# fwilliams/point-cloud-utils

Hardware: AMD Instinct MI355X
Metric: query-points/s, Chamfer 1M-vs-1M fp32 (higher is better)
Workload: dtype f32

## Files before the change

### point_cloud_utils_amd/csrc/grid.h

```cpp
#pragma once
#include "pcu_types.h"

#ifndef PCU_SORT_THREADS
#define PCU_SORT_THREADS 1024
#endif

namespace pcu {

constexpr int kBlock = 256;

template <typename T>
__device__ __forceinline__ T wave_min(T v) {
#pragma unroll
    for (int o = 32; o > 0; o >>= 1) { T w = __shfl_xor(v, o, 64); v = w < v ? w : v; }
    return v;
}
template <typename T>
__device__ __forceinline__ T wave_max(T v) {
#pragma unroll
    for (int o = 32; o > 0; o >>= 1) { T w = __shfl_xor(v, o, 64); v = w > v ? w : v; }
    return v;
}

template <int CTRL, int ROW_MASK, int BANK_MASK, bool BOUND>
// ... 389 lines not shown
template <typename T>
__global__ __launch_bounds__(kBlock) void k_scatter(const T* __restrict__ pts, int n, const unsigned* __restrict__ cell_of,
                                                    const unsigned* rank, const unsigned* __restrict__ cell_start,
                                                    Pt4<T>* __restrict__ sorted) {
    const int i = blockIdx.x * kBlock + threadIdx.x;
    if (i >= n) return;
    if (cell_of[i] == 0xffffffffu) return;
    Pt4<T> p;
    p.x = pts[3 * (size_t)i]; p.y = pts[3 * (size_t)i + 1]; p.z = pts[3 * (size_t)i + 2]; p.idx = i;
    const unsigned pos = cell_start[cell_of[i]] + rank[i];
    sorted[pos] = p;
    put_xyz(sorted, n, pos, p);
}

constexpr int kBkThreads = 1024;
#ifndef PCU_BK_PTS
#define PCU_BK_PTS 8
#endif
constexpr int kBkPts = PCU_BK_PTS;
constexpr int kBkBlockPts = kBkThreads * kBkPts;
constexpr int kBkMaxBuckets = 8192;
constexpr int kBkMaxCellsPerBucket = 4096;
constexpr int kSortThreads = PCU_SORT_THREADS;
constexpr int kSortIters = 8;
constexpr unsigned kLargeBucket = kSortThreads * kSortIters;
#ifndef PCU_BUCKET_PTS
#define PCU_BUCKET_PTS 4096
#endif
#ifndef PCU_STAGE_RECS
#define PCU_STAGE_RECS 4352
#endif
constexpr int kBucketPts = PCU_BUCKET_PTS;
constexpr int kStageRecs = PCU_STAGE_RECS;

template <typename T> struct RawRec;
template <> struct RawRec<float>  { typedef unsigned __attribute__((ext_vector_type(4))) type; };
template <> struct RawRec<double> { typedef unsigned long long __attribute__((ext_vector_type(4))) type; };

template <typename T>
__device__ __forceinline__ unsigned cell_linear(const GridParams<T>& g, T x, T y, T z) {
    const int cx = grid_cell(g, 0, x), cy = grid_cell(g, 1, y), cz = grid_cell(g, 2, z);
    return (unsigned)row_run_lo(g.G[0], grid_row(g.G[1], cy, cz), cx, cx);
}

__device__ __forceinline__ unsigned count_rank(unsigned* counter, unsigned key, bool valid) {
    const unsigned long long act = __ballot(valid);
    if (act == 0) return 0;
// ... 571 lines not shown
```

### point_cloud_utils_amd/csrc/grid2.h

```cpp
#pragma once
#include "grid.h"

namespace pcu {

constexpr int kPrepSamples = 1024;
constexpr int kXPartStride = 8;
constexpr int kStagedMaxBuckets = 2048;
constexpr int kFillWords = 2 * kStagedMaxBuckets + 8;

template <typename T>
struct CellMap {
    T org[3], inv_h; int G[3];
    __device__ __forceinline__ explicit CellMap(const GridParams<T>& g) {
#pragma unroll
        for (int j = 0; j < 3; ++j) { org[j] = uniform(g.org[j]); G[j] = uniform(g.G[j]); }
        inv_h = uniform(g.inv_h);
    }
    __device__ __forceinline__ unsigned cell(T x, T y, T z) const {
        const int cx = cell_coord(x, org[0], inv_h, G[0]), cy = cell_coord(y, org[1], inv_h, G[1]), cz = cell_coord(z, org[2], inv_h, G[2]);
        return (unsigned)row_run_lo(G[0], grid_row(G[1], cy, cz), cx, cx);
    }
};

__device__ __forceinline__ unsigned hash32(unsigned x) { x ^= x >> 16; x *= 0x7feb352du; x ^= x >> 15; x *= 0x846ca68bu; x ^= x >> 16; return x; }
// ... 189 lines not shown
            const bool valid = base + j * kBkThreads + tid < n;
            bk[j] = cm.cell(px[j], py[j], pz[j]) >> shift;
            rk[j] = count_rank(s_cnt, bk[j], valid);
            const T v[3] = {px[j], py[j], pz[j]};
#pragma unroll
            for (int c = 0; c < 3; ++c) {
                const bool fin = (v[c] < (T)0 ? -v[c] : v[c]) <= Limits<T>::max_v;
                lo[c] = (valid && fin && v[c] < lo[c]) ? v[c] : lo[c];
                hi[c] = (valid && fin && v[c] > hi[c]) ? v[c] : hi[c];
                if (valid && !fin) nf |= v[c] != v[c] ? 1u : (v[c] > (T)0 ? (2u << c) : (16u << c));
            }
        }
#pragma unroll
        for (int c = 0; c < 3; ++c) { s_col[c * kBkThreads + tid] = lo[c]; s_col[(3 + c) * kBkThreads + tid] = hi[c]; }
        const unsigned wf = wave_or63(nf);
        if (wf && lane == 63) atomicOr(&s_nf, wf);
    }
    __syncthreads();
    P3_PROF(2);
    if (wave < 6) {
        const T r = fold_column<T, kBkThreads>(s_col + wave * kBkThreads, wave < 3 ? 0 : 1, lane);
        if (lane == 63) a.xpartial[(size_t)bid * kXPartStride + wave] = r;
    } else if (tid == 6 * 64) a.xpartial[(size_t)bid * kXPartStride + 6] = (T)s_nf;
    {
        static_assert(kStagedMaxBuckets == 2 * kBkThreads, "two buckets per thread");
        const int i0 = 2 * tid;
        const unsigned c0 = i0 < NB ? s_cnt[i0] : 0u, c1 = i0 + 1 < NB ? s_cnt[i0 + 1] : 0u;
        unsigned total;
        const unsigned ex = block_exclusive_scan_nt<kBkThreads>(c0 + c1, &total);
        if (i0 < NB) s_lbase[i0] = ex;
        if (i0 + 1 < NB) s_lbase[i0 + 1] = ex + c0;
#pragma unroll
        for (int q = 0; q < 2; ++q) {
            const int i = i0 + q; const unsigned c = q ? c1 : c0;
            if (i < NB && c) {
                const unsigned pad = (c + 7u) & ~7u;
                const unsigned at = (unsigned)atomicAdd(&a.fill[i], ((unsigned long long)c << 32) | (unsigned long long)pad);
                if (at + pad > cap) { *a.ovf = 1ull; s_gbase[i] = 0xffffffffu; }
                else s_gbase[i] = (unsigned)i * cap + at;
            }
        }
    }
    __syncthreads();
    P3_PROF(3);
    typedef typename RawRec<T>::type Raw;
#pragma unroll
    for (int j = 0; j < PTS; ++j) {
        const int i = base + j * kBkThreads + tid;
        if (i < n) { Pt4<T> p; p.x = px[j]; p.y = py[j]; p.z = pz[j]; p.idx = i; s_stage[s_lbase[bk[j]] + rk[j]] = p; }
    }
    __syncthreads();
    P3_PROF(4);
    Pt4<T> hole; hole.x = hole.y = hole.z = (T)0; hole.idx = -1;
    for (int r0 = 0; r0 * 1024 + wave < NB; ++r0) {
        const int mine = wave + 16 * (64 * r0 + lane);
        const unsigned mc = mine < NB ? s_cnt[mine] : 0u, ml = mine < NB ? s_lbase[mine] : 0u, mg = mine < NB ? s_gbase[mine] : 0u;
        const int nk = min(64, (NB - wave - 1024 * r0 + 15) / 16);
        for (int k = 0; k < nk; ++k) {
            const unsigned c = (unsigned)__shfl((int)mc, k, 64);
            if (c == 0) continue;
            const unsigned lb = (unsigned)__shfl((int)ml, k, 64), gb = (unsigned)__shfl((int)mg, k, 64);
            if (gb == 0xffffffffu) continue;
            const unsigned pad = (c + 7u) & ~7u;
            for (unsigned l = (unsigned)lane; l < pad; l += 64u) {
                Pt4<T> rec = hole;
                if (l < c) rec = s_stage[lb + l];
                a.tmp[gb + l] = rec;
            }
        }
    }
    P3_PROF(5);
    if (prof) { asm volatile("s_waitcnt vmcnt(0)" ::: "memory"); P3_PROF(6); if (tid == 0) atomicAdd((unsigned long long*)&prof[15], 1ull); }
#undef P3_PROF
}

template <typename T>
__device__ __forceinline__ void fold_xpartials(const Build2Side<T>& a) {
    __shared__ T s_lo[kSortThreads / 64][3], s_hi[kSortThreads / 64][3];
    __shared__ unsigned s_nf[kSortThreads / 64];
    const int tid = threadIdx.x, lane = tid & 63, wave = tid >> 6;
    __shared__ int s_stale;
    if (tid == 0) s_stale = 0;
    if (a.geo_out) {
        extern __shared__ __attribute__((aligned(32))) unsigned char s_dyn[];
        T* const s_col = reinterpret_cast<T*>(s_dyn);
        __shared__ T s_fin[13];
        __shared__ GridParams<T> s_fresh;
        T rng6[6];
        const SampleOf<T> smp = sample_request<T>(a, a.n, tid);
        layout_from_sample<T>(a, a.n, smp, s_col, s_fin, &s_fresh, rng6);
// ... 34 lines not shown
    for (int j = 0; j < 3; ++j) {
        const T p = wave_min63(lo[j]), q = wave_max63(hi[j]);
        if (lane == 63) { s_lo[wave][j] = p; s_hi[wave][j] = q; }
    }
    { const unsigned m = wave_or63(nf); if (lane == 63) s_nf[wave] = m; }
    __syncthreads();
    if (tid != 0) return;
    GridParams<T>* gp = a.gp;
    unsigned m = 0;
    for (int w = 0; w < kSortThreads / 64; ++w) m |= s_nf[w];
    const unsigned pinf = (m >> 1) & 7u, ninf = (m >> 4) & 7u;
    gp->nonfinite = ((m & 1u) ? kNfNaN : 0) | ((pinf & ninf) ? kNfBothInf : 0) | ((pinf | ninf) ? kNfAnyInf : 0) | (int)(m << 8);
    for (int j = 0; j < 3; ++j) {
        T p = s_lo[0][j], q = s_hi[0][j];
        for (int w = 1; w < kSortThreads / 64; ++w) { p = s_lo[w][j] < p ? s_lo[w][j] : p; q = s_hi[w][j] > q ? s_hi[w][j] : q; }
        if (!(p <= q)) { p = 0; q = 0; }
        gp->gmin[j] = p; gp->gmax[j] = q;
    }
    gp->has_large = (*a.ovf ? 2 : 0) | (s_stale ? kGeoStale : 0);
    if (a.n_large) *a.n_large = 0u;
    put_sentinels(a.sorted, a.n);
}

constexpr int kRegIters = (kStageRecs + kSortThreads - 1) / kSortThreads;
template <typename T, bool FAST>
__device__ __forceinline__ void sort2_body(const int b, const Build2Side<T>& a, const int cnt_cap, const unsigned s, const unsigned pf, const unsigned nvalid,
                                           unsigned* const s_cnt, Pt4<T>* const s_stage, unsigned* const s_w, unsigned long long* const s_q, long long t_prev) {
    GridParams<T>* const gp = a.gp;
    const CellMap<T> cm(*gp);
    const int ncells = uniform(gp->ncells);
    const int shift = a.shift, CB = 1 << shift;
    const int NB = (ncells + CB - 1) >> shift;
    const int tid = threadIdx.x, lane = tid & 63, wave = tid >> 6;
    long long* const prof = a.prof;
#define S2_PROF(slot) do { if (prof && tid == 0) { const long long t_now = wall_clock64(); atomicAdd((unsigned long long*)&prof[slot], (unsigned long long)(t_now - t_prev)); t_prev = t_now; } } while (0)
    const unsigned cap = a.cap;
    const unsigned c0 = (unsigned)b << shift;
    const int ncl = min(CB, ncells - (int)c0);
    const unsigned e = s + nvalid;
    const Pt4<T>* const slot = a.tmp + (size_t)b * cap;
    const unsigned lastp = pf ? pf - 1u : 0u;
    typedef typename RawRec<T>::type Raw;
    constexpr int kIters = FAST ? kRegIters : kSortIters;
    constexpr int kSortBatch = 4;
    Raw recs[FAST ? kRegIters : 1];
    unsigned rr[kIters];
    if (FAST) {
        const Raw* const rslot = reinterpret_cast<const Raw*>(slot);
#pragma unroll
        for (int u = 0; u < kRegIters; ++u) recs[u] = rslot[min((unsigned)(u * kSortThreads + tid), lastp)];
#pragma unroll
        for (int u = 0; u < kRegIters; ++u) {
            const unsigned p = (unsigned)(u * kSortThreads + tid);
            const Pt4<T>& rec = reinterpret_cast<const Pt4<T>&>(recs[u]);
            rr[u] = 0xffffffffu;
            if (p < pf && rec.idx >= 0) {
                const unsigned c = cm.cell(rec.x, rec.y, rec.z) - c0;
                rr[u] = (c << 16) | atomicAdd(&s_cnt[c], 1u);
            }
        }
    } else {
#pragma unroll
        for (int it0 = 0; it0 < kIters; it0 += kSortBatch) {
            Pt4<T> rec[kSortBatch];
            const bool batch_on = (unsigned)(it0 * kSortThreads) < pf;
            if (batch_on) {
#pragma unroll
                for (int u = 0; u < kSortBatch; ++u) rec[u] = slot[min((unsigned)((it0 + u) * kSortThreads + tid), lastp)];
            }
#pragma unroll
            for (int u = 0; u < kSortBatch; ++u) {
                const unsigned p = (unsigned)((it0 + u) * kSortThreads + tid);
                rr[it0 + u] = 0xffffffffu;
// ... 46 lines not shown
    T* const xyz = xyz_of(a.sorted, n_pts);
    int* const idx32 = idx32_of(a.sorted, n_pts);
    if (!FAST) {
#pragma unroll
        for (int it0 = 0; it0 < kIters; it0 += kSortBatch) {
            if (!((unsigned)(it0 * kSortThreads) < pf)) break;
            Pt4<T> rec[kSortBatch];
#pragma unroll
            for (int u = 0; u < kSortBatch; ++u) rec[u] = slot[min((unsigned)((it0 + u) * kSortThreads + tid), lastp)];
#pragma unroll
            for (int u = 0; u < kSortBatch; ++u) {
                const unsigned r = rr[it0 + u];
                if (r != 0xffffffffu) {
                    const unsigned pos = s + s_cnt[r >> 16] + (r & 0xffffu);
                    if (a.want_pt4) a.sorted[pos] = rec[u];
                    put_xyz(a.sorted, n_pts, pos, rec[u]);
                }
            }
        }
        return;
    }
    constexpr unsigned V = 16 / sizeof(T);
    T* const st = reinterpret_cast<T*>(s_stage);
    int* const sidx = reinterpret_cast<int*>(st + (V + 3 * kStageRecs + V - 1) / V * V);
    static_assert(((V + 3 * kStageRecs + V - 1) / V * V) * sizeof(T) + (size_t)kStageRecs * 4 <= (size_t)kStageRecs * sizeof(Pt4<T>) + 64, "both streams fit the stage (bucket_sort_lds_bytes)");
    const unsigned phase = (unsigned)((3ull * (unsigned long long)s) & (V - 1));
    {
#pragma unroll
        for (int u = 0; u < kRegIters; ++u) {
            const unsigned r = rr[u];
            if (r != 0xffffffffu) {
                const Pt4<T>& rec = reinterpret_cast<const Pt4<T>&>(recs[u]);
                const unsigned pos = s_cnt[r >> 16] + (r & 0xffffu);
                T* const o = st + phase + 3u * pos;
                o[0] = rec.x; o[1] = rec.y; o[2] = rec.z; sidx[pos] = (int)rec.idx;
            }
        }
    }
    __syncthreads();
    S2_PROF(3);
    for (unsigned i = tid; i < nvalid; i += kSortThreads) {
        const int id = sidx[i];
        idx32[s + i] = id;
        if (a.want_pt4) { Pt4<T> r; const T* const o = st + phase + 3u * i; r.x = o[0]; r.y = o[1]; r.z = o[2]; r.idx = id; a.sorted[s + i] = r; }
    }
    {
        const unsigned end = phase + 3u * nvalid;
        T* const out = xyz + (3 * (size_t)s - phase);
        typedef typename RawRec<float>::type Raw16;
        const unsigned v0 = (phase + V - 1) / V, v1 = end / V;
        for (unsigned c = v0 + tid; c < v1; c += kSortThreads)
            reinterpret_cast<Raw16*>(out)[c] = reinterpret_cast<const Raw16*>(st)[c];
        if (tid < V) {
            const unsigned La = phase + tid;
            if (La < min(v0 * V, end)) out[La] = st[La];
            const unsigned Lb = max(v1 * V, v0 * V) + tid;
            if (v1 >= v0 && Lb < end) out[Lb] = st[Lb];
        }
    }
    S2_PROF(4);
    if (prof) { asm volatile("s_waitcnt vmcnt(0)" ::: "memory"); S2_PROF(5); if (tid == 0) atomicAdd((unsigned long long*)&prof[7], 1ull); }
#undef S2_PROF
}

template <typename T>
__device__ __forceinline__ void sort2_bucket(const int b, const Build2Side<T>& a, const int cnt_cap) {
    extern __shared__ __attribute__((aligned(32))) unsigned char s_dyn[];
    unsigned* const s_cnt = reinterpret_cast<unsigned*>(s_dyn);
    Pt4<T>* const s_stage = reinterpret_cast<Pt4<T>*>(s_dyn + (size_t)cnt_cap * 4);
    __shared__ unsigned s_w[kSortThreads / 64 + 1];
    __shared__ unsigned long long s_q[kSortThreads / 64];
    if (*a.ovf) return;
    const int CB = 1 << a.shift;
    const int NB = (uniform(a.gp->ncells) + CB - 1) >> a.shift;
    if (b >= NB) return;
    const int tid = threadIdx.x, lane = tid & 63, wave = tid >> 6;
    long long t_prev = a.prof ? wall_clock64() : 0;
    unsigned s;
    {
        unsigned part = 0;
        for (int i = tid; i < b; i += kSortThreads) part += (unsigned)(a.fill[i] >> 32);
#pragma unroll
        for (int o = 32; o > 0; o >>= 1) part += __shfl_xor(part, o, 64);
        if (lane == 0) s_w[wave] = part;
        for (int i = tid; i < CB; i += kSortThreads) s_cnt[i] = 0u;
        __syncthreads();
        s = 0;
        for (int w = 0; w < kSortThreads / 64; ++w) s += s_w[w];
        __syncthreads();
    }
    if (a.prof && tid == 0) { const long long t_now = wall_clock64(); atomicAdd((unsigned long long*)&a.prof[0], (unsigned long long)(t_now - t_prev)); t_prev = t_now; }
    const unsigned long long fw = a.fill[b];
    const unsigned pf = min((unsigned)fw, a.cap), nvalid = (unsigned)(fw >> 32);
    static_assert(kSortThreads * kSortIters >= kLargeBucket, "one trip per record of a full slot");
    if (pf <= (unsigned)(kRegIters * kSortThreads) && nvalid <= (unsigned)kStageRecs) sort2_body<T, true>(b, a, cnt_cap, s, pf, nvalid, s_cnt, s_stage, s_w, s_q, t_prev);
    else sort2_body<T, false>(b, a, cnt_cap, s, pf, nvalid, s_cnt, s_stage, s_w, s_q, t_prev);
}

template <typename T>
__global__ __launch_bounds__(kSortThreads) void k_bucket_sort2(const Build2Args<T> p, int nb0, int nb1, int cnt_cap, int nfold) {
    const int bid = (int)blockIdx.x;
    if (bid < nfold) { fold_xpartials<T>(p.a[bid]); return; }
    const int b = bid - nfold;
    const int side = b >= nb0 ? 1 : 0;
    sort2_bucket<T>(side ? b - nb0 : b, p.a[side], cnt_cap);
}

template <typename T>
struct Pt4Side { Pt4<T>* sorted; int n; };
template <typename T>
__global__ __launch_bounds__(kBlock) void k_make_pt4(const Pt4Side<T> a0, const Pt4Side<T> a1, int nb0) {
    const bool second = (int)blockIdx.x >= nb0;
    const Pt4Side<T>& a = second ? a1 : a0;
    const int nblk = second ? (int)gridDim.x - nb0 : nb0, bid = second ? (int)blockIdx.x - nb0 : (int)blockIdx.x;
    const T* const xyz = xyz_of(a.sorted, a.n);
    const int* const idx32 = idx32_of(a.sorted, a.n);
    for (int i = bid * kBlock + (int)threadIdx.x; i < a.n + 8; i += nblk * kBlock) {
        Pt4<T> r; r.x = xyz[3 * (size_t)i]; r.y = xyz[3 * (size_t)i + 1]; r.z = xyz[3 * (size_t)i + 2]; r.idx = idx32[i];
        a.sorted[i] = r;
// ... 5 lines not shown
```

### point_cloud_utils_amd/csrc/pcu_hip.hip

```cpp
#include <hip/hip_runtime.h>
#include <math.h>
#include <stdarg.h>
#include <stdio.h>
#include <string.h>
#include <stdlib.h>
#include <stddef.h>
#include <algorithm>
#include <limits>
#include <string>
#include <vector>
#include <chrono>
#include <atomic>
#include <signal.h>
#include <time.h>

#include "../../include/pcu_hip.h"
#include "grid.h"
#include "grid2.h"
#include "reduce.h"
#include "search.h"
namespace pcu {
#define PCU_SEARCH_INST extern template
#include "search_inst.h"
#undef PCU_SEARCH_INST
// ... 1563 lines not shown
    PairState<T> P;
    Arena ar; Timer tm; hipStream_t s = nullptr;
    const T *x = nullptr, *y = nullptr; int64_t nx = 0, ny = 0;
    bool on_dev = false; unsigned flags = 0; pcu_hip_stats* st = nullptr;
    int restarts = 0;
    bool squared = false, two_sided = true; int max_leaf = 10;
    bool tie_xy = false, tie_yx = false; int fuse_mode = FUSE_NONE;
    double p_norm = 2.0; int64_t *out_cxy = nullptr, *out_cyx = nullptr;
};
template <typename T>
static size_t pair_bytes(int64_t nx, int64_t ny, double occ_x, double occ_y, bool on_dev) {
    size_t b = index_bytes<T>(std::max(nx, ny), occ_x) + index_bytes<T>(std::max(nx, ny), occ_y) + scratch_bytes<T>(nx) + scratch_bytes<T>(ny) +
               align_up((size_t)nx * sizeof(T), 256) + align_up((size_t)ny * sizeof(T), 256) +
               align_up((size_t)nx * 8, 256) + align_up((size_t)ny * 8, 256) +
               6 * align_up((size_t)kRedBlocks * 8, 256) + 8192 +
               3 * (align_up((size_t)grid8((int)nx, kBlock) * 8, 256) + align_up((size_t)grid8((int)ny, kBlock) * 8, 256)) +
               4 * align_up((size_t)kWaveBlocks * (kBlock / 64) * 8, 256) + align_up(sizeof(CallBlock), 256) + 1024;
    if (!on_dev) b += align_up((size_t)nx * 3 * sizeof(T), 256) + align_up((size_t)ny * 3 * sizeof(T), 256) +
                      align_up((size_t)nx * 8, 256) + align_up((size_t)ny * 8, 256);
    return b;
}
static int wait_result_block(pcu_hip_ctx* c, hipStream_t s);
template <typename T>
static int pair_search_enqueue(pcu_hip_ctx* c, hipStream_t s, PairState<T>& P, pcu_hip_stats* st) {
    const bool lazy_wave = P.fuse && P.two && lane_k1_job(P.xy) && lane_k1_job(P.yx);
    if (P.two) { if (search_enqueue_pair(c, s, P.xy, P.yx, st, lazy_wave ? 1 : 3)) return -1; }
    else if (search_enqueue(c, s, P.xy, st, false)) return -1;
    P.wave_pending = lazy_wave;
    if (P.fuse) {
        P.tail.nwaves = lazy_wave ? 0 : kWaveBlocks * (kBlock / 64);
        hipLaunchKernelGGL(k_fuse_tail<T>, dim3(1), dim3(kTailThreads), 0, s, P.tail);
        HIP_TRY(hipGetLastError());
    }
    return 0;
}
template <typename T>
static int fused_wave_if_needed(pcu_hip_ctx* c, hipStream_t s, PairState<T>& P, pcu_hip_stats* st, ResultBlock& host, Fused& out) {
    if ((host.counters[0][C_LARGE] | (P.two ? host.counters[1][C_LARGE] : 0)) & kGeoStale) { c->geo.valid[0] = c->geo.valid[1] = false; out = Fused::Restart; return 0; }
    if (!P.wave_pending) return 0;
    P.wave_pending = false;
    bool need = false, broken = false;
    for (int d = 0; d < 2; ++d) {
        need = need || host.counters[d][C_U1] > 0 || host.counters[d][C_T1] > 0;
        broken = broken || host.counters[d][C_SKEW] || host.counters[d][C_LARGE];
    }
    if (!need || broken) return 0;
    if (search_enqueue_pair(c, s, P.xy, P.yx, st, 2)) return -1;
    P.tail.nwaves = kWaveBlocks * (kBlock / 64); P.tail.seq = ++c->seq;
    hipLaunchKernelGGL(k_fuse_tail<T>, dim3(1), dim3(kTailThreads), 0, s, P.tail);
    HIP_TRY(hipGetLastError());
    if (wait_result_block(c, s)) return -1;
    memcpy(&host, c->h_pinned, sizeof host);
    return 0;
}
template <typename T>
static int pair_setup(pcu_hip_ctx* c, PendingPair<T>& pp, double occ_x, double occ_y) {
    PairState<T>& P = pp.P; Arena& ar = pp.ar; Timer& tm = pp.tm; hipStream_t s = pp.s; pcu_hip_stats* st = pp.st;
    const int64_t nx = pp.nx, ny = pp.ny; const bool two_sided = pp.two_sided, squared = pp.squared; const int fuse_mode = pp.fuse_mode;
    long long* const ext_ixy = pp.on_dev ? (long long*)pp.out_cxy : nullptr; long long* const ext_iyx = pp.on_dev ? (long long*)pp.out_cyx : nullptr;
    P.two = two_sided;
    P.xy.leaf_max = P.yx.leaf_max = pp.max_leaf > 0 ? pp.max_leaf : 10; P.xy.tie_order = pp.tie_xy; P.yx.tie_order = pp.tie_yx;
    if (stage_in(ar, pp.x, nx, pp.on_dev, s, &P.dx)) return -1;
    if (stage_in(ar, pp.y, ny, pp.on_dev, s, &P.dy)) return -1;
    GridIndex<T> ix, iy;
    const bool share = two_sided && shared_grid_wanted(c, nx, ny, occ_x, occ_y);
    const int64_t n_plan = share ? std::max(nx, ny) : 0;
    if (index_alloc(ar, ix, nx, occ_x, true, use_one_pass(c), n_plan) || index_alloc(ar, iy, ny, occ_y, true, use_one_pass(c), n_plan)) return -1;
    ix.shared_grid = iy.shared_grid = share;
    ix.src = P.dx; iy.src = P.dy; ix.occ_built = occ_x; iy.occ_built = occ_y;
    if (ix.bucketed && iy.bucketed && ix.one_pass != iy.one_pass) ix.one_pass = iy.one_pass = false;
    P.xy.qidx = ix; P.xy.ridx = iy; P.xy.d_ref_pts = P.dy;
    P.yx.qidx = iy; P.yx.ridx = ix; P.yx.d_ref_pts = P.dx;
// ... 93 lines not shown
static bool fused_rescale(pcu_hip_ctx* c, hipStream_t s, const PairState<T>& P, const ResultBlock& h) {
    bool want = false;
    for (int d = 0; d < (P.two ? 2 : 1) && !want; ++d)
        if (h.counters[d][C_SKEW]) want = rescale_wanted(c, d ? P.yx : P.xy, s, h.counters[d][C_SKEW]);
    return want;
}
template <typename T>
static int fused_continue(pcu_hip_ctx* c, Arena& ar, hipStream_t s, PairState<T>& P, pcu_hip_stats* st, ResultBlock& host, bool tie_matters, Fused& out) {
    static const bool off = getenv("PCU_HIP_NO_FUSED_CONTINUE") != nullptr;
    out = Fused::Rows; if (off) return 0;
    const int nd = P.two ? 2 : 1;
    bool any = false;
    for (int d = 0; d < nd; ++d) {
        if (host.counters[d][C_SKEW] || host.counters[d][C_LARGE]) return 0;
        any = any || host.counters[d][C_U2] > 0;
    }
    if (!any) return 0;
    for (int d = 0; d < nd; ++d) {
        if (host.counters[d][C_U2] <= 0) { if (st) { st->n_escalated += host.counters[d][C_U1]; st->n_tie_flagged += host.counters[d][C_T1]; } continue; }
        Outcome fin;
        if (int r = search_finish(c, ar, s, d ? P.yx : P.xy, st, host.counters[d], fin)) return r;
    }
    P.tail.seq = ++c->seq;
    hipLaunchKernelGGL(k_fuse_tail<T>, dim3(1), dim3(kTailThreads), 0, s, P.tail);
    HIP_TRY(hipGetLastError());
    if (wait_result_block(c, s)) return -1;
    memcpy(&host, c->h_pinned, sizeof host);
    if (fused_ok(P, host, tie_matters, true)) out = Fused::Done;
    return 0;
}
template <typename T>
static int pair_unlean(hipStream_t s, PairState<T>& P) {
    if (int rc = unlean(s, P.xy.qidx, P.xy.ridx)) return rc;
    P.yx.qidx.lean = P.yx.ridx.lean = false;
    return 0;
}
template <typename T>
static int pair_nonfinite_flags(hipStream_t s, const PairState<T>& P, int (&nf)[2]) {
    const GridParams<T>* gp[2] = {P.xy.qidx.gp, P.xy.ridx.gp};
    for (int d = 0; d < 2; ++d)
        HIP_TRY(hipMemcpyAsync(&nf[d], reinterpret_cast<const char*>(gp[d]) + offsetof(GridParams<T>, nonfinite), sizeof(int), hipMemcpyDeviceToHost, s));
    HIP_WAIT(s);
    return 0;
}
template <typename T>
static int unfuse_and_research(pcu_hip_ctx* c, hipStream_t s, PairState<T>& P, pcu_hip_stats* st, bool skip_search = false) {
    P.fuse = FUSE_NONE; P.xy.fuse = P.yx.fuse = FUSE_NONE;
// ... 737 lines not shown
```

### point_cloud_utils_amd/csrc/pcu_types.h

```cpp
#pragma once
#include <hip/hip_runtime.h>
#include <stdint.h>
#include <float.h>

namespace pcu {

template <typename T> struct Pt4;
template <> struct alignas(16) Pt4<float>  { float x, y, z; int idx; };
template <> struct alignas(32) Pt4<double> { double x, y, z; long long idx; };

template <typename T> __host__ __device__ __forceinline__ T* xyz_of(Pt4<T>* sorted, int n) { return reinterpret_cast<T*>(sorted + n + 8); }
template <typename T> __host__ __device__ __forceinline__ const T* xyz_of(const Pt4<T>* sorted, int n) { return reinterpret_cast<const T*>(sorted + n + 8); }
template <typename T> __host__ __device__ __forceinline__ int* idx32_of(Pt4<T>* sorted, int n) { return reinterpret_cast<int*>(xyz_of(sorted, n) + 3 * (size_t)(n + 8)); }
template <typename T> __host__ __device__ __forceinline__ const int* idx32_of(const Pt4<T>* sorted, int n) { return reinterpret_cast<const int*>(xyz_of(sorted, n) + 3 * (size_t)(n + 8)); }
template <typename T> __device__ __forceinline__ void put_xyz(Pt4<T>* sorted, int n, unsigned pos, const Pt4<T>& r) {
    T* o = xyz_of(sorted, n) + 3 * (size_t)pos;
    o[0] = r.x; o[1] = r.y; o[2] = r.z;
    idx32_of(sorted, n)[pos] = (int)r.idx;
}
template <typename T> __device__ __forceinline__ void put_sentinels(Pt4<T>* sorted, int n) {
    for (int j = 0; j < 8; ++j) {
        Pt4<T> s; s.x = s.y = s.z = (T)INFINITY; s.idx = 0x7fffffff;
        sorted[n + j] = s;
        put_xyz(sorted, n, (unsigned)(n + j), s);
    }
}
constexpr size_t sorted_records_bytes(size_t n, size_t rec_bytes, size_t scalar_bytes) { return (n + 8) * (rec_bytes + 3 * scalar_bytes + 4); }

__device__ __forceinline__ bool cancel_seen(const unsigned* word, unsigned gen) {
    return word != nullptr && (int)(__hip_atomic_load(word, __ATOMIC_RELAXED, __HIP_MEMORY_SCOPE_SYSTEM) - gen) > 0;
}

__device__ __forceinline__ int uniform(int v) { return __builtin_amdgcn_readfirstlane(v); }
__device__ __forceinline__ float uniform(float v) { return __int_as_float(__builtin_amdgcn_readfirstlane(__float_as_int(v))); }
__device__ __forceinline__ unsigned long long uniform(unsigned long long v) {
    const unsigned lo = (unsigned)__builtin_amdgcn_readfirstlane((int)(unsigned)v), hi = (unsigned)__builtin_amdgcn_readfirstlane((int)(unsigned)(v >> 32));
    return ((unsigned long long)hi << 32) | lo;
}
__device__ __forceinline__ double uniform(double v) { return __longlong_as_double((long long)uniform((unsigned long long)__double_as_longlong(v))); }

template <typename T> struct Limits;
template <> struct Limits<float>  { static constexpr float  max_v = FLT_MAX; static constexpr float  eps = FLT_EPSILON; };
template <> struct Limits<double> { static constexpr double max_v = DBL_MAX; static constexpr double eps = DBL_EPSILON; };

__device__ __forceinline__ unsigned int enc(float f) {
    unsigned int u = __float_as_uint(f);
    return (u & 0x80000000u) ? ~u : (u | 0x80000000u);
}
__device__ __forceinline__ float dec(unsigned int u) {
    return __uint_as_float((u & 0x80000000u) ? (u & 0x7fffffffu) : ~u);
}
__device__ __forceinline__ unsigned long long enc(double f) {
    unsigned long long u = (unsigned long long)__double_as_longlong(f);
    return (u & 0x8000000000000000ull) ? ~u : (u | 0x8000000000000000ull);
}
__device__ __forceinline__ double dec(unsigned long long u) {
    return __longlong_as_double((long long)((u & 0x8000000000000000ull) ? (u & 0x7fffffffffffffffull) : ~u));
}
template <typename T> struct EncT;
template <> struct EncT<float>  { using type = unsigned int; };
template <> struct EncT<double> { using type = unsigned long long; };

template <typename T>
struct GridParams {
    T gmin[3], gmax[3];
// ... 44 lines not shown
```

### point_cloud_utils_amd/csrc/reduce.h

```cpp
#pragma once
#include "pcu_types.h"
#include "grid.h"

namespace pcu {

constexpr int kRedBlocks = 1024;
#ifndef PCU_RED_BLOCKS
#define PCU_RED_BLOCKS 128
#endif
constexpr int kRedBlocksFused = PCU_RED_BLOCKS;

template <typename T>
__device__ __forceinline__ void argmax_combine(T& v, long long& i, T v2, long long i2) {
    if (v2 > v || (v2 == v && i2 < i)) { v = v2; i = i2; }
}

template <typename T>
struct ArgmaxSide { const T* d; const long long* corr; int n; int nb; };

template <typename T>
__device__ __forceinline__ void block_argmax(T& v, long long& idx) {
#pragma unroll
    for (int o = 32; o > 0; o >>= 1) {
        T v2 = __shfl_xor(v, o, 64); long long i2 = __shfl_xor(idx, o, 64);
// ... 135 lines not shown
__device__ __forceinline__ double tail_sum(const double (&v)[kTailLanes / NT], double* s_buf) {
    constexpr int V = kTailLanes / NT;
    double w[V];
#pragma unroll
    for (int q = 0; q < V; ++q) {
        w[q] = v[q];
#pragma unroll
        for (int o = 32; o > 0; o >>= 1) w[q] += __shfl_xor(w[q], o, 64);
    }
    __syncthreads();
    if ((threadIdx.x & 63) == 0) {
#pragma unroll
        for (int q = 0; q < V; ++q) s_buf[q * (NT / 64) + (threadIdx.x >> 6)] = w[q];
    }
    __syncthreads();
    double r = s_buf[0];
    for (int i = 1; i < kTailLanes / 64; ++i) r += s_buf[i];
    return r;
}
struct VK { double v; long long k; };
__device__ __forceinline__ VK comb_max(VK a, VK b) { return (b.v > a.v || (b.v == a.v && b.k < a.k)) ? b : a; }
__device__ __forceinline__ VK shfl_vk(VK a, int o) { VK r; r.v = __shfl_xor(a.v, o, 64); r.k = __shfl_xor(a.k, o, 64); return r; }

template <typename T, int NT>
__device__ __forceinline__ void fuse_tail_body(const FuseTail<T>& ft) {
    __shared__ double s_d[kTailLanes / 64]; __shared__ double s_mv[NT / 64]; __shared__ long long s_mk[NT / 64];
    __shared__ int s_res[64]; __shared__ unsigned long long s_mask;
    constexpr int kTailThreads = NT, V = kTailLanes / NT;
    const int tid = threadIdx.x;
    long long t_prev = ft.prof ? wall_clock64() : 0;
#define TAIL_PROF(slot) do { if (ft.prof && tid == 0) { const long long t_now = wall_clock64(); atomicAdd((unsigned long long*)&ft.prof[slot], (unsigned long long)(t_now - t_prev)); t_prev = t_now; } } while (0)
    const int rbw = tid < 63 ? ft.result_block[tid] : 0;
    double acc[2][V];
#pragma unroll
    for (int q = 0; q < V; ++q) { acc[0][q] = 0; acc[1][q] = 0; }
    VK best[2] = {{-DBL_MAX, 0x7fffffffffffffffll}, {-DBL_MAX, 0x7fffffffffffffffll}};
#pragma unroll
    for (int jb = 0; jb < 2; ++jb) {
        if (jb >= ft.njobs) continue;
        if (ft.mode == FUSE_SUM) {
            constexpr int kBatch = 8;
            const double* const fs = ft.flat_sum[jb]; const int nf = ft.nflat[jb];
            for (int b0 = 0; b0 < nf; b0 += kBatch * kTailLanes) {
                double v[V][kBatch];
#pragma unroll
                for (int q = 0; q < V; ++q)
#pragma unroll
                    for (int u = 0; u < kBatch; ++u) { const int i = b0 + u * kTailLanes + tid + q * NT; v[q][u] = i < nf ? fs[i] : 0.0; }
#pragma unroll
                for (int q = 0; q < V; ++q)
#pragma unroll
                    for (int u = 0; u < kBatch; ++u) acc[jb][q] += v[q][u];
            }
#pragma unroll
            for (int q = 0; q < V; ++q) { const int vt = tid + q * NT; if (vt <= kAccLimbs) acc[jb][q] += exact_term(ft.limbs[jb], ft.special[jb], vt); }
        } else {
            constexpr int kBatch = 8;
            const T* const fv = ft.flat_v[jb]; const long long* const fk = ft.flat_k[jb]; const int nf = ft.nflat[jb];
            for (int b0 = tid; b0 < nf; b0 += kBatch * kTailThreads) {
                T v[kBatch]; long long k[kBatch];
#pragma unroll
                for (int u = 0; u < kBatch; ++u) { const int i = min(b0 + u * kTailThreads, nf - 1); v[u] = fv[i]; k[u] = fk[i]; }
#pragma unroll
                for (int u = 0; u < kBatch; ++u) { const VK c = {(double)v[u], k[u]}; best[jb] = comb_max(best[jb], c); }
            }
            const T* const wv = ft.wave_v[jb]; const long long* const wk = ft.wave_k[jb];
            for (int b0 = tid; b0 < ft.nwaves; b0 += kBatch * kTailThreads) {
                T v[kBatch]; long long k[kBatch];
#pragma unroll
                for (int u = 0; u < kBatch; ++u) {
                    const int i = min(b0 + u * kTailThreads, ft.nwaves - 1);
                    v[u] = wv[i]; k[u] = wk[i];
                }
#pragma unroll
                for (int u = 0; u < kBatch; ++u) { const VK c = {(double)v[u], k[u]}; best[jb] = comb_max(best[jb], c); }
            }
        }
    }
    TAIL_PROF(0);
    if (tid == 0) s_mask = 0ull;
    if (ft.mode == FUSE_SUM && V == 1) {
        __shared__ double s_ws[2][kTailLanes / 64];
        double w[2] = {acc[0][0], acc[1][0]};
#pragma unroll
        for (int jb = 0; jb < 2; ++jb) {
#pragma unroll
            for (int o = 32; o > 0; o >>= 1) w[jb] += __shfl_xor(w[jb], o, 64);
        }
        __syncthreads();
        if ((tid & 63) == 0) { s_ws[0][tid >> 6] = w[0]; s_ws[1][tid >> 6] = w[1]; }
        __syncthreads();
        if (tid == 0) {
#pragma unroll
            for (int jb = 0; jb < 2; ++jb) {
                if (jb >= ft.njobs) continue;
                double r = s_ws[jb][0];
                for (int i = 1; i < kTailLanes / 64; ++i) r += s_ws[jb][i];
                *reinterpret_cast<double*>(&s_res[ft.w_sums + 2 * jb]) = r; s_mask |= 3ull << (ft.w_sums + 2 * jb);
            }
        }
    } else if (ft.mode == FUSE_SUM) {
#pragma unroll
        for (int jb = 0; jb < 2; ++jb) {
            if (jb >= ft.njobs) continue;
            const double r = tail_sum<NT>(acc[jb], s_d);
            if (tid == 0) { *reinterpret_cast<double*>(&s_res[ft.w_sums + 2 * jb]) = r; s_mask |= 3ull << (ft.w_sums + 2 * jb); }
        }
    } else {
        VK win[2] = {best[0], best[1]};
        __shared__ double s_wv[2][NT / 64]; __shared__ long long s_wk[2][NT / 64]; __shared__ double s_fv[2]; __shared__ long long s_fk[2];
        static_assert(NT / 64 == 16, "16 wave winners per direction");
#pragma unroll
        for (int jb = 0; jb < 2; ++jb) {
#pragma unroll
            for (int o = 32; o > 0; o >>= 1) win[jb] = comb_max(win[jb], shfl_vk(win[jb], o));
        }
        if ((tid & 63) == 0) {
#pragma unroll
            for (int jb = 0; jb < 2; ++jb) { s_wv[jb][tid >> 6] = win[jb].v; s_wk[jb][tid >> 6] = win[jb].k; }
        }
        __syncthreads();
        if (tid < 32) {
            const int jb = tid >> 4, w = tid & 15;
            VK v = {s_wv[jb][w], s_wk[jb][w]};
// ... 23 lines not shown
        TAIL_PROF(2);
        if (tid == 0) {
#pragma unroll
            for (int jb = 0; jb < 2; ++jb) {
                if (jb >= ft.njobs) continue;
                const VK v = win[jb];
                const int wv = ft.w_vals + jb * (int)(sizeof(T) / 4), wi = ft.w_ij + 4 * jb, wt = ft.w_tie + jb;
                *reinterpret_cast<T*>(&s_res[wv]) = (T)v.v; s_mask |= (sizeof(T) == 8 ? 3ull : 1ull) << wv;
                *reinterpret_cast<long long*>(&s_res[wi]) = v.k >> 32; *reinterpret_cast<long long*>(&s_res[wi + 2]) = v.k & 0x7fffffffll; s_mask |= 15ull << wi;
                s_res[wt] = (int)((v.k >> 31) & 1ll); s_mask |= 1ull << wt;
            }
        }
    }
    __syncthreads();
    TAIL_PROF(3);
    if (ft.prof && tid == 0) atomicAdd((unsigned long long*)&ft.prof[7], 1ull);
#undef TAIL_PROF
    if (tid < 64) {
        if (tid < 63) ft.host_block[tid] = ((s_mask >> tid) & 1ull) ? s_res[tid] : rbw;
        __threadfence_system();
        if (tid == 63) __hip_atomic_store(&ft.host_block[63], (int)ft.seq, __ATOMIC_RELAXED, __HIP_MEMORY_SCOPE_SYSTEM);
    }
}
template <typename T>
__global__ __launch_bounds__(1024) void k_fuse_tail(const FuseTail<T> ft) { fuse_tail_body<T, 1024>(ft); }

template <typename T>
__global__ __launch_bounds__(kBlock) void k_tie_hit(const int* __restrict__ tt, int n, const Pt4<T>* __restrict__ qsorted,
                                                    const long long* __restrict__ ij, int* flag) {
    const long long row = ij[0];
    for (int i = blockIdx.x * kBlock + threadIdx.x; i < n; i += gridDim.x * kBlock)
        if ((long long)qsorted[tt[i]].idx == row) *flag = 1;
}

__device__ __forceinline__ double block_sum(double s) {
#pragma unroll
    for (int o = 32; o > 0; o >>= 1) s += __shfl_xor(s, o, 64);
    __shared__ double ss[kBlock / 64];
    if ((threadIdx.x & 63) == 0) ss[threadIdx.x >> 6] = s;
    __syncthreads();
    double r = 0;
    if (threadIdx.x == 0) for (int w = 0; w < kBlock / 64; ++w) r += ss[w];
    return r;
}

enum { P_TWO = 0, P_ONE = 1, P_INF = 2, P_NINF = 3, P_ZERO = 4, P_GEN = 5 };

template <typename T>
// ... 77 lines not shown
```

Before: 16.63 billion.

## Defer bucket-fill atomics, use 16-byte write-through stores, specialize fuse tail by mode

Bucket-claim atomic results are now consumed only after the LDS staging loop, so the atomic latency overlaps that work. Scatter and sort-output copies now go through 16-byte chunked stores with the sc1 cache hint, and the sorted index stream is also written vectorized with phase alignment. The prefix-of-fill loads for the sort head are issued before the register record loads and folded afterwards. The fused tail kernel is templated on mode to remove runtime branching. Several unrelated tweaks are bundled, and the inline-asm stores skip compiler scheduling and depend on the sc1 hint behaving as intended.

```diff
diff --git a/point_cloud_utils_amd/csrc/grid.h b/point_cloud_utils_amd/csrc/grid.h
--- a/point_cloud_utils_amd/csrc/grid.h
+++ b/point_cloud_utils_amd/csrc/grid.h
@@ -435,7 +435,10 @@
 constexpr int kBkMaxBuckets = 8192;
 constexpr int kBkMaxCellsPerBucket = 4096;
 constexpr int kSortThreads = PCU_SORT_THREADS;
-constexpr int kSortIters = 8;
+#ifndef PCU_SORT_ITERS
+#define PCU_SORT_ITERS 8
+#endif
+constexpr int kSortIters = PCU_SORT_ITERS;
 constexpr unsigned kLargeBucket = kSortThreads * kSortIters;
 #ifndef PCU_BUCKET_PTS
 #define PCU_BUCKET_PTS 4096
diff --git a/point_cloud_utils_amd/csrc/grid2.h b/point_cloud_utils_amd/csrc/grid2.h
--- a/point_cloud_utils_amd/csrc/grid2.h
+++ b/point_cloud_utils_amd/csrc/grid2.h
@@ -235,10 +235,12 @@
         const T r = fold_column<T, kBkThreads>(s_col + wave * kBkThreads, wave < 3 ? 0 : 1, lane);
         if (lane == 63) a.xpartial[(size_t)bid * kXPartStride + wave] = r;
     } else if (tid == 6 * 64) a.xpartial[(size_t)bid * kXPartStride + 6] = (T)s_nf;
+    unsigned long long at[2] = {0ull, 0ull}; unsigned rc0, rc1;
     {
         static_assert(kStagedMaxBuckets == 2 * kBkThreads, "two buckets per thread");
         const int i0 = 2 * tid;
         const unsigned c0 = i0 < NB ? s_cnt[i0] : 0u, c1 = i0 + 1 < NB ? s_cnt[i0 + 1] : 0u;
+        rc0 = c0; rc1 = c1;
         unsigned total;
         const unsigned ex = block_exclusive_scan_nt<kBkThreads>(c0 + c1, &total);
         if (i0 < NB) s_lbase[i0] = ex;
@@ -246,25 +248,32 @@
 #pragma unroll
         for (int q = 0; q < 2; ++q) {
             const int i = i0 + q; const unsigned c = q ? c1 : c0;
-            if (i < NB && c) {
-                const unsigned pad = (c + 7u) & ~7u;
-                const unsigned at = (unsigned)atomicAdd(&a.fill[i], ((unsigned long long)c << 32) | (unsigned long long)pad);
-                if (at + pad > cap) { *a.ovf = 1ull; s_gbase[i] = 0xffffffffu; }
-                else s_gbase[i] = (unsigned)i * cap + at;
-            }
+            if (i < NB && c) at[q] = atomicAdd(&a.fill[i], ((unsigned long long)c << 32) | (unsigned long long)((c + 7u) & ~7u));
         }
     }
     __syncthreads();
     P3_PROF(3);
-    typedef typename RawRec<T>::type Raw;
 #pragma unroll
     for (int j = 0; j < PTS; ++j) {
         const int i = base + j * kBkThreads + tid;
         if (i < n) { Pt4<T> p; p.x = px[j]; p.y = py[j]; p.z = pz[j]; p.idx = i; s_stage[s_lbase[bk[j]] + rk[j]] = p; }
     }
+    asm volatile("" :: "v"(at[0]), "v"(at[1]));
+#pragma unroll
+    for (int q = 0; q < 2; ++q) {
+        const int i = 2 * tid + q; const unsigned c = q ? rc1 : rc0;
+        if (i < NB && c) {
+            const unsigned pad = (c + 7u) & ~7u, lo = (unsigned)at[q];
+            if (lo + pad > cap) { *a.ovf = 1ull; s_gbase[i] = 0xffffffffu; }
+            else s_gbase[i] = (unsigned)i * cap + lo;
+        }
+    }
     __syncthreads();
     P3_PROF(4);
-    Pt4<T> hole; hole.x = hole.y = hole.z = (T)0; hole.idx = -1;
+    constexpr unsigned CH = sizeof(Pt4<T>) / 16;
+    const Chunk16* const stage16 = reinterpret_cast<const Chunk16*>(s_stage);
+    Chunk16* const tmp16 = reinterpret_cast<Chunk16*>(a.tmp);
+    const Chunk16 zero16 = {0u, 0u, 0u, 0u}, hole_id16 = {0u, 0u, sizeof(T) == 8 ? 0xffffffffu : 0u, 0xffffffffu};
     for (int r0 = 0; r0 * 1024 + wave < NB; ++r0) {
         const int mine = wave + 16 * (64 * r0 + lane);
         const unsigned mc = mine < NB ? s_cnt[mine] : 0u, ml = mine < NB ? s_lbase[mine] : 0u, mg = mine < NB ? s_gbase[mine] : 0u;
@@ -275,10 +284,10 @@
             const unsigned lb = (unsigned)__shfl((int)ml, k, 64), gb = (unsigned)__shfl((int)mg, k, 64);
             if (gb == 0xffffffffu) continue;
             const unsigned pad = (c + 7u) & ~7u;
-            for (unsigned l = (unsigned)lane; l < pad; l += 64u) {
-                Pt4<T> rec = hole;
-                if (l < c) rec = s_stage[lb + l];
-                a.tmp[gb + l] = rec;
+            for (unsigned l = (unsigned)lane; l < pad * CH; l += 64u) {
+                Chunk16 v = (l % CH) == CH - 1 ? hole_id16 : zero16;
+                if (l / CH < c) v = stage16[(size_t)lb * CH + l];
+                store16_wt(tmp16 + ((size_t)gb * CH + l), v);
             }
         }
     }
@@ -359,9 +368,31 @@
     put_sentinels(a.sorted, a.n);
 }
 
+constexpr int kHeadTrips = (kStagedMaxBuckets + kSortThreads - 1) / kSortThreads;
+template <typename T>
+__device__ __forceinline__ void sort2_head_request(const Build2Side<T>& a, const int b, unsigned long long (&fw)[kHeadTrips]) {
+#pragma unroll
+    for (int q = 0; q < kHeadTrips; ++q) { const int i = q * kSortThreads + (int)threadIdx.x; fw[q] = i < b ? a.fill[i] : 0ull; }
+}
+__device__ __forceinline__ unsigned sort2_head_fold(const unsigned long long (&fw)[kHeadTrips], unsigned* const s_cnt, const int CB, unsigned* const s_w) {
+    const int tid = threadIdx.x, lane = tid & 63, wave = tid >> 6;
+    unsigned part = 0;
+#pragma unroll
+    for (int q = 0; q < kHeadTrips; ++q) part += (unsigned)(fw[q] >> 32);
+#pragma unroll
+    for (int o = 32; o > 0; o >>= 1) part += __shfl_xor(part, o, 64);
+    if (lane == 0) s_w[wave] = part;
+    for (int i = tid; i < CB; i += kSortThreads) s_cnt[i] = 0u;
+    __syncthreads();
+    unsigned s = 0;
+    for (int w = 0; w < kSortThreads / 64; ++w) s += s_w[w];
+    __syncthreads();
+    return s;
+}
+
 constexpr int kRegIters = (kStageRecs + kSortThreads - 1) / kSortThreads;
 template <typename T, bool FAST>
-__device__ __forceinline__ void sort2_body(const int b, const Build2Side<T>& a, const int cnt_cap, const unsigned s, const unsigned pf, const unsigned nvalid,
+__device__ __forceinline__ void sort2_body(const int b, const Build2Side<T>& a, const int cnt_cap, const unsigned long long (&hw)[kHeadTrips], const unsigned pf, const unsigned nvalid,
                                            unsigned* const s_cnt, Pt4<T>* const s_stage, unsigned* const s_w, unsigned long long* const s_q, long long t_prev) {
     GridParams<T>* const gp = a.gp;
     const CellMap<T> cm(*gp);
@@ -374,7 +405,6 @@
     const unsigned cap = a.cap;
     const unsigned c0 = (unsigned)b << shift;
     const int ncl = min(CB, ncells - (int)c0);
-    const unsigned e = s + nvalid;
     const Pt4<T>* const slot = a.tmp + (size_t)b * cap;
     const unsigned lastp = pf ? pf - 1u : 0u;
     typedef typename RawRec<T>::type Raw;
@@ -386,6 +416,11 @@
         const Raw* const rslot = reinterpret_cast<const Raw*>(slot);
 #pragma unroll
         for (int u = 0; u < kRegIters; ++u) recs[u] = rslot[min((unsigned)(u * kSortThreads + tid), lastp)];
+    }
+    const unsigned s = sort2_head_fold(hw, s_cnt, CB, s_w);
+    const unsigned e = s + nvalid;
+    S2_PROF(0);
+    if (FAST) {
 #pragma unroll
         for (int u = 0; u < kRegIters; ++u) {
             const unsigned p = (unsigned)(u * kSortThreads + tid);
@@ -478,9 +513,11 @@
     }
     constexpr unsigned V = 16 / sizeof(T);
     T* const st = reinterpret_cast<T*>(s_stage);
-    int* const sidx = reinterpret_cast<int*>(st + (V + 3 * kStageRecs + V - 1) / V * V);
-    static_assert(((V + 3 * kStageRecs + V - 1) / V * V) * sizeof(T) + (size_t)kStageRecs * 4 <= (size_t)kStageRecs * sizeof(Pt4<T>) + 64, "both streams fit the stage (bucket_sort_lds_bytes)");
+    int* const sidx0 = reinterpret_cast<int*>(st + (V + 3 * kStageRecs + V - 1) / V * V);
+    static_assert(((V + 3 * kStageRecs + V - 1) / V * V) * sizeof(T) + ((size_t)kStageRecs + 4) * 4 <= (size_t)kStageRecs * sizeof(Pt4<T>) + 64, "both streams fit the stage (bucket_sort_lds_bytes)");
     const unsigned phase = (unsigned)((3ull * (unsigned long long)s) & (V - 1));
+    const unsigned iph = (unsigned)((reinterpret_cast<size_t>(idx32 + s) >> 2) & 3u);
+    int* const sidx = sidx0 + iph;
     {
 #pragma unroll
         for (int u = 0; u < kRegIters; ++u) {
@@ -495,23 +532,34 @@
     }
     __syncthreads();
     S2_PROF(3);
-    for (unsigned i = tid; i < nvalid; i += kSortThreads) {
-        const int id = sidx[i];
-        idx32[s + i] = id;
-        if (a.want_pt4) { Pt4<T> r; const T* const o = st + phase + 3u * i; r.x = o[0]; r.y = o[1]; r.z = o[2]; r.idx = id; a.sorted[s + i] = r; }
+    if (a.want_pt4) {
+        for (unsigned i = tid; i < nvalid; i += kSortThreads) { Pt4<T> r; const T* const o = st + phase + 3u * i; r.x = o[0]; r.y = o[1]; r.z = o[2]; r.idx = sidx[i]; a.sorted[s + i] = r; }
     }
     {
         const unsigned end = phase + 3u * nvalid;
         T* const out = xyz + (3 * (size_t)s - phase);
-        typedef typename RawRec<float>::type Raw16;
         const unsigned v0 = (phase + V - 1) / V, v1 = end / V;
         for (unsigned c = v0 + tid; c < v1; c += kSortThreads)
-            reinterpret_cast<Raw16*>(out)[c] = reinterpret_cast<const Raw16*>(st)[c];
+            store16_wt(reinterpret_cast<Chunk16*>(out) + c, reinterpret_cast<const Chunk16*>(st)[c]);
         if (tid < V) {
             const unsigned La = phase + tid;
             if (La < min(v0 * V, end)) out[La] = st[La];
             const unsigned Lb = max(v1 * V, v0 * V) + tid;
             if (v1 >= v0 && Lb < end) out[Lb] = st[Lb];
+        }
+    }
+    {
+        const unsigned iend = iph + nvalid;
+        int* const iout = idx32 + s - iph;
+        const unsigned w0 = (iph + 3u) / 4u, w1 = iend / 4u;
+        for (unsigned c = w0 + tid; c < w1; c += kSortThreads)
+            store16_wt(reinterpret_cast<Chunk16*>(iout) + c, reinterpret_cast<const Chunk16*>(sidx0)[c]);
+        if (tid >= 64 && tid < 68) {
+            const unsigned t = (unsigned)tid - 64u;
+            const unsigned La = iph + t;
+            if (La < min(w0 * 4u, iend)) iout[La] = sidx0[La];
+            const unsigned Lb = max(w1 * 4u, w0 * 4u) + t;
+            if (w1 >= w0 && Lb < iend) iout[Lb] = sidx0[Lb];
         }
     }
     S2_PROF(4);
@@ -530,27 +578,14 @@
     const int CB = 1 << a.shift;
     const int NB = (uniform(a.gp->ncells) + CB - 1) >> a.shift;
     if (b >= NB) return;
-    const int tid = threadIdx.x, lane = tid & 63, wave = tid >> 6;
     long long t_prev = a.prof ? wall_clock64() : 0;
-    unsigned s;
-    {
-        unsigned part = 0;
-        for (int i = tid; i < b; i += kSortThreads) part += (unsigned)(a.fill[i] >> 32);
-#pragma unroll
-        for (int o = 32; o > 0; o >>= 1) part += __shfl_xor(part, o, 64);
-        if (lane == 0) s_w[wave] = part;
-        for (int i = tid; i < CB; i += kSortThreads) s_cnt[i] = 0u;
-        __syncthreads();
-        s = 0;
-        for (int w = 0; w < kSortThreads / 64; ++w) s += s_w[w];
-        __syncthreads();
-    }
-    if (a.prof && tid == 0) { const long long t_now = wall_clock64(); atomicAdd((unsigned long long*)&a.prof[0], (unsigned long long)(t_now - t_prev)); t_prev = t_now; }
     const unsigned long long fw = a.fill[b];
-    const unsigned pf = min((unsigned)fw, a.cap), nvalid = (unsigned)(fw >> 32);
+    unsigned long long hw[kHeadTrips];
+    sort2_head_request<T>(a, b, hw);
+    const unsigned pf = min((unsigned)uniform(fw), a.cap), nvalid = (unsigned)(uniform(fw) >> 32);
     static_assert(kSortThreads * kSortIters >= kLargeBucket, "one trip per record of a full slot");
-    if (pf <= (unsigned)(kRegIters * kSortThreads) && nvalid <= (unsigned)kStageRecs) sort2_body<T, true>(b, a, cnt_cap, s, pf, nvalid, s_cnt, s_stage, s_w, s_q, t_prev);
-    else sort2_body<T, false>(b, a, cnt_cap, s, pf, nvalid, s_cnt, s_stage, s_w, s_q, t_prev);
+    if (pf <= (unsigned)(kRegIters * kSortThreads) && nvalid <= (unsigned)kStageRecs) sort2_body<T, true>(b, a, cnt_cap, hw, pf, nvalid, s_cnt, s_stage, s_w, s_q, t_prev);
+    else sort2_body<T, false>(b, a, cnt_cap, hw, pf, nvalid, s_cnt, s_stage, s_w, s_q, t_prev);
 }
 
 template <typename T>
diff --git a/point_cloud_utils_amd/csrc/pcu_hip.hip b/point_cloud_utils_amd/csrc/pcu_hip.hip
--- a/point_cloud_utils_amd/csrc/pcu_hip.hip
+++ b/point_cloud_utils_amd/csrc/pcu_hip.hip
@@ -1609,6 +1609,11 @@
 }
 static int wait_result_block(pcu_hip_ctx* c, hipStream_t s);
 template <typename T>
+static void fuse_tail_launch(hipStream_t s, const FuseTail<T>& t) {
+    if (t.mode == FUSE_SUM) hipLaunchKernelGGL((k_fuse_tail<T, FUSE_SUM>), dim3(1), dim3(kTailThreads), 0, s, t);
+    else hipLaunchKernelGGL((k_fuse_tail<T, FUSE_ARGMAX>), dim3(1), dim3(kTailThreads), 0, s, t);
+}
+template <typename T>
 static int pair_search_enqueue(pcu_hip_ctx* c, hipStream_t s, PairState<T>& P, pcu_hip_stats* st) {
     const bool lazy_wave = P.fuse && P.two && lane_k1_job(P.xy) && lane_k1_job(P.yx);
     if (P.two) { if (search_enqueue_pair(c, s, P.xy, P.yx, st, lazy_wave ? 1 : 3)) return -1; }
@@ -1616,7 +1621,7 @@
     P.wave_pending = lazy_wave;
     if (P.fuse) {
         P.tail.nwaves = lazy_wave ? 0 : kWaveBlocks * (kBlock / 64);
-        hipLaunchKernelGGL(k_fuse_tail<T>, dim3(1), dim3(kTailThreads), 0, s, P.tail);
+        fuse_tail_launch<T>(s, P.tail);
         HIP_TRY(hipGetLastError());
     }
     return 0;
@@ -1634,7 +1639,7 @@
     if (!need || broken) return 0;
     if (search_enqueue_pair(c, s, P.xy, P.yx, st, 2)) return -1;
     P.tail.nwaves = kWaveBlocks * (kBlock / 64); P.tail.seq = ++c->seq;
-    hipLaunchKernelGGL(k_fuse_tail<T>, dim3(1), dim3(kTailThreads), 0, s, P.tail);
+    fuse_tail_launch<T>(s, P.tail);
     HIP_TRY(hipGetLastError());
     if (wait_result_block(c, s)) return -1;
     memcpy(&host, c->h_pinned, sizeof host);
@@ -1774,7 +1779,7 @@
         if (int r = search_finish(c, ar, s, d ? P.yx : P.xy, st, host.counters[d], fin)) return r;
     }
     P.tail.seq = ++c->seq;
-    hipLaunchKernelGGL(k_fuse_tail<T>, dim3(1), dim3(kTailThreads), 0, s, P.tail);
+    fuse_tail_launch<T>(s, P.tail);
     HIP_TRY(hipGetLastError());
     if (wait_result_block(c, s)) return -1;
     memcpy(&host, c->h_pinned, sizeof host);
diff --git a/point_cloud_utils_amd/csrc/pcu_types.h b/point_cloud_utils_amd/csrc/pcu_types.h
--- a/point_cloud_utils_amd/csrc/pcu_types.h
+++ b/point_cloud_utils_amd/csrc/pcu_types.h
@@ -39,8 +39,13 @@
 }
 __device__ __forceinline__ double uniform(double v) { return __longlong_as_double((long long)uniform((unsigned long long)__double_as_longlong(v))); }
 
+typedef unsigned __attribute__((ext_vector_type(4))) Chunk16;
+__device__ __forceinline__ void store16_wt(void* p, const Chunk16 v) {
+    asm volatile("global_store_dwordx4 %0, %1, off sc1\n\ts_nop 1" :: "v"(p), "v"(v));
+}
+
 template <typename T> struct Limits;
-template <> struct Limits<float>  { static constexpr float  max_v = FLT_MAX; static constexpr float  eps = FLT_EPSILON; };
+template <> struct Limits<float> { static constexpr float  max_v = FLT_MAX; static constexpr float  eps = FLT_EPSILON; };
 template <> struct Limits<double> { static constexpr double max_v = DBL_MAX; static constexpr double eps = DBL_EPSILON; };
 
 __device__ __forceinline__ unsigned int enc(float f) {
diff --git a/point_cloud_utils_amd/csrc/reduce.h b/point_cloud_utils_amd/csrc/reduce.h
--- a/point_cloud_utils_amd/csrc/reduce.h
+++ b/point_cloud_utils_amd/csrc/reduce.h
@@ -181,8 +181,9 @@
 __device__ __forceinline__ VK comb_max(VK a, VK b) { return (b.v > a.v || (b.v == a.v && b.k < a.k)) ? b : a; }
 __device__ __forceinline__ VK shfl_vk(VK a, int o) { VK r; r.v = __shfl_xor(a.v, o, 64); r.k = __shfl_xor(a.k, o, 64); return r; }
 
-template <typename T, int NT>
+template <typename T, int NT, int MODE>
 __device__ __forceinline__ void fuse_tail_body(const FuseTail<T>& ft) {
+    static_assert(MODE == FUSE_SUM || MODE == FUSE_ARGMAX, "the two fused epilogues");
     __shared__ double s_d[kTailLanes / 64]; __shared__ double s_mv[NT / 64]; __shared__ long long s_mk[NT / 64];
     __shared__ int s_res[64]; __shared__ unsigned long long s_mask;
     constexpr int kTailThreads = NT, V = kTailLanes / NT;
@@ -197,7 +198,7 @@
 #pragma unroll
     for (int jb = 0; jb < 2; ++jb) {
         if (jb >= ft.njobs) continue;
-        if (ft.mode == FUSE_SUM) {
+        if (MODE == FUSE_SUM) {
             constexpr int kBatch = 8;
             const double* const fs = ft.flat_sum[jb]; const int nf = ft.nflat[jb];
             for (int b0 = 0; b0 < nf; b0 += kBatch * kTailLanes) {
@@ -238,7 +239,7 @@
     }
     TAIL_PROF(0);
     if (tid == 0) s_mask = 0ull;
-    if (ft.mode == FUSE_SUM && V == 1) {
+    if (MODE == FUSE_SUM && V == 1) {
         __shared__ double s_ws[2][kTailLanes / 64];
         double w[2] = {acc[0][0], acc[1][0]};
 #pragma unroll
@@ -258,7 +259,7 @@
                 *reinterpret_cast<double*>(&s_res[ft.w_sums + 2 * jb]) = r; s_mask |= 3ull << (ft.w_sums + 2 * jb);
             }
         }
-    } else if (ft.mode == FUSE_SUM) {
+    } else if (MODE == FUSE_SUM) {
 #pragma unroll
         for (int jb = 0; jb < 2; ++jb) {
             if (jb >= ft.njobs) continue;
@@ -328,8 +329,8 @@
         if (tid == 63) __hip_atomic_store(&ft.host_block[63], (int)ft.seq, __ATOMIC_RELAXED, __HIP_MEMORY_SCOPE_SYSTEM);
     }
 }
-template <typename T>
-__global__ __launch_bounds__(1024) void k_fuse_tail(const FuseTail<T> ft) { fuse_tail_body<T, 1024>(ft); }
+template <typename T, int MODE>
+__global__ __launch_bounds__(1024) void k_fuse_tail(const FuseTail<T> ft) { fuse_tail_body<T, 1024, MODE>(ft); }
 
 template <typename T>
 __global__ __launch_bounds__(kBlock) void k_tie_hit(const int* __restrict__ tt, int n, const Pt4<T>* __restrict__ qsorted,
```

Result: faster. 17.20 billion (median of 6 runs) (+3.5%).
